# kohjingyu/gill

Hardware: AMD Instinct MI355X
Metric: 512x512 images/sec/node, OPT-6.7B+SD1.5 50-step (higher is better)
Workload: dtype bf16

## Files before the change

### gill_amd/csrc/attention.hip

```cpp
#include "ops.h"
#include <stdlib.h>
#include <type_traits>

#define ATT_KVT 64

template <int DP, int ATT_THREADS>
struct AttCfg {
  static constexpr int KS = DP / 16;
  static constexpr int NDT = (DP + 31) / 32;
  static constexpr int DPV = NDT * 32;
  static constexpr int KSTR = DP + 8;
  static constexpr int VSTR = ATT_KVT + 8;
  static constexpr bool HAS_ONES = (DP % 32) != 0;
  static constexpr int K_CHUNKS = ATT_KVT * DP / 8;
  static constexpr int V_CHUNKS = DPV * ATT_KVT / 8;
  static constexpr int K_PER_THR = (K_CHUNKS + ATT_THREADS - 1) / ATT_THREADS;
  static constexpr int V_PER_THR = (V_CHUNKS + ATT_THREADS - 1) / ATT_THREADS;
  static constexpr int K_ROWS = (K_PER_THR * ATT_THREADS + DP / 8 - 1) / (DP / 8);
  static constexpr int V_ROWS = K_PER_THR * 0 + V_PER_THR * ATT_THREADS / 8;
  static constexpr int K_ELEMS = K_ROWS * KSTR;
  static constexpr int V_ELEMS = V_ROWS * VSTR;
  static constexpr int BUF_ELEMS = K_ELEMS + V_ELEMS;
  static constexpr int SMEM_BYTES = 2 * BUF_ELEMS * 2;
};

template <int DP, int ATT_THREADS>
__global__ __launch_bounds__(ATT_THREADS, (DP <= 64 ? 4 : 2)) void attention_kernel(const AttnArgs p) {
  kernarg_warm<sizeof(AttnArgs)>();
  using Cfg = AttCfg<DP, ATT_THREADS>;
  constexpr int ATT_QB = ATT_THREADS / 2;
  constexpr int KS = Cfg::KS, NDT = Cfg::NDT, KSTR = Cfg::KSTR, VSTR = Cfg::VSTR;
  extern __shared__ __attribute__((aligned(16))) unsigned char att_smem_raw[];
  bf16_t* smem = reinterpret_cast<bf16_t*>(att_smem_raw);

  const int tid = threadIdx.x;
  const int lane = tid & 63;
  const int w = tid >> 6;
  const int nqt = (p.nq + ATT_QB - 1) / ATT_QB;
  int pair, qtile;
  if (p.xcd_map) {
    const int xcd = blockIdx.x & 7, slot = blockIdx.x >> 3;
    pair = xcd + 8 * (slot / nqt);
    qtile = slot - (slot / nqt) * nqt;
  } else {
    pair = blockIdx.x / nqt;
    qtile = blockIdx.x - pair * nqt;
  }
  if (pair >= p.B * p.H) return;
  const int b = pair / p.H, h = pair - b * p.H;
  const int q0 = qtile * ATT_QB + w * 32;
  const bool wave_active = q0 < p.nq;
  const int lq = lane & 31;
  const int hi = lane >> 5;
  const int kvb = p.kv_bstride_zero ? 0 : b;

  const bf16_t* Qb = p.Q + (size_t)(b * p.H + h) * p.nq_pad * DP;
  const bf16_t* Kb = p.K + (size_t)(kvb * p.H + h) * p.nkv_pad * DP;
  const bf16_t* Vb = p.Vt + (size_t)(kvb * p.H + h) * p.dpv * p.nkv_pad;

  int qrow = q0 + lq;
  const bool qvalid = qrow < p.nq;
  if (qrow > p.nq - 1) qrow = p.nq - 1;

  bf16x8 qf[KS];
#pragma unroll
  for (int s = 0; s < KS; ++s) qf[s] = *reinterpret_cast<const bf16x8*>(Qb + (size_t)qrow * DP + s * 16 + hi * 8);

  f32x16 oacc[NDT];
#pragma unroll
  for (int t = 0; t < NDT; ++t)
#pragma unroll
    for (int r = 0; r < 16; ++r) oacc[t][r] = 0.f;

  float m_run = 0.f, l_run = 0.f;

  const int coff = p.nkv - p.nq;
  int kv_end_blk = p.nkv;
  if (p.causal) {
    int lim = qtile * ATT_QB + ATT_QB - 1 + coff + 1;
    if (lim < kv_end_blk) kv_end_blk = lim;
    if (kv_end_blk < 1) kv_end_blk = 1;
  }
  const int ntiles = (kv_end_blk + ATT_KVT - 1) / ATT_KVT;
  const int qidx = qrow + coff;
  const int wave_kv_end = p.causal ? min(p.nkv, q0 + 31 + coff + 1) : p.nkv;

  typedef __attribute__((ext_vector_type(4))) unsigned int u32x4;
  u32x4 kreg[Cfg::K_PER_THR];
  u32x4 vreg[Cfg::V_PER_THR];
// ... 164 lines not shown

template <int DP, int ATT_THREADS>
__global__ __launch_bounds__(ATT_THREADS, 4) void attention_dma_kernel(const AttnArgs p) {
  kernarg_warm<sizeof(AttnArgs)>();
  static_assert(DP == 48, "QF3 needs three padding dims behind d = 40");
  constexpr int NW = ATT_THREADS / 64;
  constexpr int ATT_QB = ATT_THREADS / 2;
  constexpr int KS = DP / 16, NDT = (DP + 31) / 32, NCH = DP / 8;
  constexpr int PPW = 8 / NW;
  constexpr int K_BYTES = 64 * 128, STAGE = 2 * K_BYTES, CONST_OFF = 2 * STAGE;
  extern __shared__ __attribute__((aligned(16))) unsigned char att_smem_raw[];
  unsigned char* smem = att_smem_raw;

  const int tid = threadIdx.x;
  const int lane = tid & 63;
  const int w = __builtin_amdgcn_readfirstlane(tid >> 6);
  const int nqt = p.nq / ATT_QB;
  int pair, qtile;
  if (p.xcd_map) {
    const int xcd = blockIdx.x & 7, slot = blockIdx.x >> 3;
    pair = xcd + 8 * (slot / nqt);
    qtile = slot - (slot / nqt) * nqt;
  } else {
    pair = blockIdx.x / nqt;
    qtile = blockIdx.x - pair * nqt;
  }
  if (pair >= p.B * p.H) return;
  const int b = pair / p.H, h = pair - b * p.H;
  const int q0 = qtile * ATT_QB + w * 32;
  const int lq = lane & 31;
  const int hi = lane >> 5;
  const int kvb = p.kv_bstride_zero ? 0 : b;

  const bf16_t* Qb = p.Q + (size_t)(b * p.H + h) * p.nq_pad * DP;
  const bf16_t* Kb = p.K + (size_t)(kvb * p.H + h) * p.nkv_pad * DP;
  const bf16_t* Vb = p.Vt + (size_t)(kvb * p.H + h) * p.dpv * p.nkv_pad;
  const int qrow = q0 + lq;

  if (tid == 0) *reinterpret_cast<uint4*>(smem + CONST_OFF) = make_uint4(0x3F803F80u, 0x00003F80u, 0u, 0u);

  bf16x8 qf[KS];
#pragma unroll
  for (int s = 0; s < KS; ++s) qf[s] = *reinterpret_cast<const bf16x8*>(Qb + (size_t)qrow * DP + s * 16 + hi * 8);

  const int r8 = lane >> 3, pch = lane & 7;
  unsigned koff[PPW], voff[PPW];
#pragma unroll
  for (int j = 0; j < PPW; ++j) {
    const int i = (w * PPW + j) * 8 + r8;
    const int c = pch ^ ((i >> 1) & 7);
    const int key = (i & ~12) | ((i & 4) << 1) | ((i & 8) >> 1);
    const int ck = c >= NCH ? c - NCH : c;
    koff[j] = (unsigned)((key * DP + ck * 8) * 2);
    voff[j] = (unsigned)((i * p.nkv_pad + c * 8) * 2);
  }
  auto issue_tile = [&](int tile, int stage) {
    const char* kbase = (const char*)(Kb + (size_t)tile * ATT_KVT * DP);
    const char* vbase = (const char*)(Vb + (size_t)tile * ATT_KVT);
    unsigned char* dst = smem + stage * STAGE + (w * PPW) * 1024;
#pragma unroll
    for (int j = 0; j < PPW; ++j) {
      __builtin_amdgcn_global_load_lds((const __attribute__((address_space(1))) void*)(kbase + koff[j]),
                                       (__attribute__((address_space(3))) void*)(dst + j * 1024), 16, 0, 0);
      __builtin_amdgcn_global_load_lds((const __attribute__((address_space(1))) void*)(vbase + voff[j]),
                                       (__attribute__((address_space(3))) void*)(dst + K_BYTES + j * 1024), 16, 0, 0);
    }
  };
// ... 157 lines not shown
static int attention_launch_inst(const AttnArgs& a, hipStream_t s) {
  static bool attr_set = false;
  constexpr int smem = AttCfg<DP, NTHR>::SMEM_BYTES;
  if (!attr_set) {
    GILL_CHECK_HIP(hipFuncSetAttribute((const void*)attention_kernel<DP, NTHR>, hipFuncAttributeMaxDynamicSharedMemorySize, smem));
    attr_set = true;
  }
  constexpr int xcd_on = 1;
  AttnArgs b = a;
  b.xcd_map = xcd_on;
  dim3 grid((xcd_on ? 8 * cdiv(a.H * a.B, 8) : a.H * a.B) * cdiv(a.nq, NTHR / 2), 1, 1);
  hipLaunchKernelGGL((attention_kernel<DP, NTHR>), grid, dim3(NTHR), smem, s, b);
  GILL_CHECK_HIP(hipGetLastError());
  return 0;
}

template <int DP>
static int attention_launch_dp(const AttnArgs& a, hipStream_t s) {
  const int64_t bh = (int64_t)a.H * a.B;
  const bool big = cdiv(a.nq, 256) * bh >= 256;
  if constexpr (DP == 48) {
    if (attention_dma_ok(a, big ? 512 : 256)) return big ? attention_dma_launch<DP, 512>(a, s) : attention_dma_launch<DP, 256>(a, s);
  }
  if (big) return attention_launch_inst<DP, 512>(a, s);
  return attention_launch_inst<DP, 256>(a, s);
}

int attention_launch(const AttnArgs& a, hipStream_t s) {
  GILL_REQUIRE(a.B > 0 && a.H > 0 && a.nq > 0 && a.nkv > 0, "empty attention");
  GILL_REQUIRE(a.nkv_pad % 32 == 0 && a.nkv_pad >= a.nkv, "nkv_pad must be a multiple of 32 covering nkv");
  GILL_REQUIRE(a.nq_pad >= a.nq, "nq_pad must cover nq");
  GILL_REQUIRE(a.dpv >= round_up(a.dp, 32), "dpv must cover roundup(dp, 32)");
  GILL_REQUIRE(a.ldo >= a.H * a.dp, "ldo too small");
  switch (a.dp) {
    case 48:  return attention_launch_dp<48>(a, s);
    case 64:  return attention_launch_dp<64>(a, s);
    case 80:  return attention_launch_dp<80>(a, s);
    case 128: return attention_launch_dp<128>(a, s);
    case 160: return attention_launch_dp<160>(a, s);
    default:
      gill_set_error("attention: unsupported padded head dim (supported: 48, 64, 80, 128, 160)");
      return -2;
  }
}
```

### gill_amd/csrc/ffn.hip

```cpp
#include "ops.h"
#include <type_traits>

namespace {

constexpr int FC = 320;
constexpr int FH = 1280;
constexpr int FTM = 128;
constexpr int FSLOT = 20 * 1024;
constexpr int FNSLOT = 7;
constexpr int FNCH = FH / 64;
constexpr int FBIAS_OFF = FNSLOT * FSLOT;
constexpr int FBO2_OFF = FBIAS_OFF + FNCH * 128 * 4;
constexpr int FW_BYTES = 2560;
constexpr int FSMEM = FBIAS_OFF + FNCH * 128 * 4;
constexpr int FSMEM_PRE = FBO2_OFF + FC * 4;
static_assert(FSMEM_PRE <= 160 * 1024, "LDS budget");
constexpr int FKO = 384;
constexpr int FNPRE = 2 * (FKO / 64);

typedef __attribute__((ext_vector_type(16))) float f32x16;
typedef __attribute__((ext_vector_type(4))) float f32x4;
typedef __attribute__((ext_vector_type(4))) unsigned u32x4;
typedef __attribute__((ext_vector_type(2))) unsigned u32x2;

template <int N> __device__ __forceinline__ void ffn_wait_vm() {
  __builtin_amdgcn_s_waitcnt((N & 15) | ((N >> 4) << 14) | (7 << 4) | (15 << 8));
}

struct Slab { const bf16_t* src; int ld; };

template <bool PRE>
__global__ __launch_bounds__(256) __attribute__((amdgpu_waves_per_eu(1, 1))) void ffn_fused_kernel(const FfnArgs p) {
  kernarg_warm<sizeof(FfnArgs)>();
  constexpr int SB = PRE ? FNPRE % 7 : 0;
  extern __shared__ __attribute__((aligned(16))) unsigned char smem[];
  const int tid = threadIdx.x, lane = tid & 63;
  const int w = __builtin_amdgcn_readfirstlane(tid >> 6);
  const int l31 = lane & 31, hi = lane >> 5;
  const int m = blockIdx.x * FTM + w * 32 + l31;

  const int srow = lane >> 3, schunk = (lane & 7) ^ srow;
  auto slab_f = [&](int f) -> Slab {
    if constexpr (PRE) return Slab{p.Wpp + (size_t)(f / 5) * 160 * FC + 64 * (f % 5), FC};
    else return Slab{p.Wfo + (size_t)(f / 5) * 160 * (5 * FC) + 4 * FC + 64 * (f % 5), 5 * FC};
  };
  auto slab_g = [&](int g) -> Slab { return Slab{p.Wo + (size_t)(g / 6) * 160 * FKO + 64 * (g % 6), FKO}; };
  auto slab_c = [&](int c, int q) -> Slab {
    if (q < 5) return Slab{p.W1c + (size_t)c * 128 * FC + 64 * q, FC};
    return Slab{p.W2p + (size_t)(q - 5) * 160 * FH + 64 * c, FH};
  };
  auto issue_piece = [&](const Slab& st, int slot, int i) {
    const int pc = w + 4 * i;
    const uint64_t b64 = (uint64_t)(uintptr_t)(st.src + (size_t)(8 * pc) * st.ld);
    const bf16_t* base = (const bf16_t*)(uintptr_t)(((uint64_t)(unsigned)__builtin_amdgcn_readfirstlane((unsigned)(b64 >> 32)) << 32) |
                                                     (uint64_t)(unsigned)__builtin_amdgcn_readfirstlane((unsigned)b64));
    const bf16_t* src = (const bf16_t*)((const char*)base + (unsigned)((srow * st.ld + schunk * 8) * 2));
    __builtin_amdgcn_global_load_lds((const __attribute__((address_space(1))) void*)src,
                                     (__attribute__((address_space(3))) void*)(smem + slot * FSLOT + pc * 1024), 16, 0, 0);
  };
  auto wfrag = [&](const unsigned char* slot, int tile, int s) -> bf16x8 {
    const int row = tile * 32 + l31;
    return *reinterpret_cast<const bf16x8*>(slot + row * 128 + (((2 * s + hi) ^ (row & 7)) * 16));
  };

#pragma unroll
  for (int f = 0; f < 6; ++f) {
    const Slab st = PRE ? slab_g(f) : slab_f(f);
#pragma unroll
    for (int i = 0; i < 5; ++i) issue_piece(st, f, i);
  }
  __builtin_amdgcn_sched_barrier(0);
  bf16x8 tf[20];
  float ln_mean, ln_rstd;
  bf16x8 xf[PRE ? FKO / 16 : 1];
  u32x4 res[PRE ? 20 : 1];
  if constexpr (PRE) {
    const bf16_t* tsrc = p.T + (size_t)(blockIdx.x * FTM + w * 32 + (lane >> 2)) * FC + (lane & 3) * 8;
#pragma unroll
    for (int i = 0; i < 10; ++i) {
      res[2 * i] = *reinterpret_cast<const u32x4*>(tsrc + 32 * i);
      res[2 * i + 1] = *reinterpret_cast<const u32x4*>(tsrc + 32 * i + 16 * FC);
    }
#pragma unroll
    for (int s = 0; s < FKO / 16; ++s) xf[s] = *reinterpret_cast<const bf16x8*>(p.X + (size_t)m * FKO + 16 * s + 8 * hi);
  } else {
#pragma unroll
    for (int s = 0; s < 20; ++s) tf[s] = *reinterpret_cast<const bf16x8*>(p.T + (size_t)m * FC + 16 * s + 8 * hi);
    const int R = p.ln_rows ? p.ln_rows : p.M;
    const int mr = m >= R ? m - R : m;
    const float* base = p.ln_stats + (size_t)mr * 2;
    const size_t pstride = (size_t)R * 2;
    float2 st = make_float2(0.f, 0.f);
    for (int pl = 0; pl < p.ln_planes; ++pl) {
      const float2 v = *reinterpret_cast<const float2*>(base + (size_t)pl * pstride);
      st.x += v.x; st.y += v.y;
    }
    ln_mean = st.x * (1.f / FC);
    const float var = fmaxf(st.y * (1.f / FC) - ln_mean * ln_mean, 0.f);
    ln_rstd = rsqrtf(var + p.ln_eps);
  }
  {
    float* bt = reinterpret_cast<float*>(smem + FBIAS_OFF);
    static_assert(FNCH * 128 % 256 == 0, "table fill: whole rounds of the workgroup");
    float tb[FNCH * 128 / 256];
#pragma unroll
    for (int j = 0; j < FNCH * 128 / 256; ++j) tb[j] = p.b1c[tid + 256 * j];
#pragma unroll
    for (int j = 0; j < FNCH * 128 / 256; ++j) bt[tid + 256 * j] = tb[j];
    if constexpr (PRE) {
      float* b2t = reinterpret_cast<float*>(smem + FBO2_OFF);
// ... 176 lines not shown
          const f32x4 bg = *reinterpret_cast<const f32x4*>(btab + c * 128 + 64 + tt * 32 + 16 * hh + 8 * g2 + 4 * hi);
          const int r = 8 * hh + 4 * g2;
          const float o0 = (acc[tt][r] + bv.x) * gelu_logistic(acc[2 + tt][r] + bg.x);
          const float o1 = (acc[tt][r + 1] + bv.y) * gelu_logistic(acc[2 + tt][r + 1] + bg.y);
          const float o2 = (acc[tt][r + 2] + bv.z) * gelu_logistic(acc[2 + tt][r + 2] + bg.z);
          const float o3 = (acc[tt][r + 3] + bv.w) * gelu_logistic(acc[2 + tt][r + 3] + bg.w);
          pk.u[2 * g2] = pack_bf2(o0, o1);
          pk.u[2 * g2 + 1] = pack_bf2(o2, o3);
        }
        pf[2 * tt + hh] = pk.v;
      }
#define S2_STAGE(U, N, NL)                                                                                                      \
    {                                                                                                                            \
      auto mma = [&](int s, const bf16x8* wfp) {                                                                                 \
        _Pragma("unroll") for (int q = 0; q < 5; ++q)                                                                           \
          out[5 * (U) + q] = __builtin_amdgcn_mfma_f32_32x32x16_bf16(wfp[q], pf[s], out[5 * (U) + q], 0, 0, 0);                  \
      };                                                                                                                         \
      const Slab nx = slab_c(LAST ? c : c + 1, 4 + (U));                                                                         \
      run_stage(I5{}, std::integral_constant<int, (U) == 0 ? 5 : (LAST ? 0 : 4)>{}, std::integral_constant<int, LAST ? NL : N>{},\
                std::integral_constant<int, LAST ? 0 : ((U) == 1 ? 5 : 4)>{}, (SB + 8 + (U)) % 7, (SB + 9 + (U)) % 7, nx,        \
                (SB + 7 + (U)) % 7, mma, std::false_type{});                                                                     \
    }
    S2_STAGE(0, 19, 0) S2_STAGE(1, 19, 0)
#undef S2_STAGE
  };
  for (int c = 0; c + 1 < FNCH; ++c) run_chunk(c, std::false_type{});
  run_chunk(FNCH - 1, std::true_type{});

  constexpr int OSTR = 656;
  __syncthreads();
  unsigned char* wtile = smem + (size_t)(w * 32) * OSTR;
  unsigned char* otile = wtile + (size_t)l31 * OSTR;
  {
    const bf16_t* rsrc = p.resid + (size_t)(blockIdx.x * FTM + w * 32) * FC;
    u32x4 rr[20];
#pragma unroll
    for (int j = 0; j < 20; ++j) rr[j] = *reinterpret_cast<const u32x4*>(rsrc + (size_t)(lane + 64 * j) * 8);
#pragma unroll
    for (int j = 0; j < 20; ++j) {
      const int c = lane + 64 * j;
      *reinterpret_cast<u32x4*>(wtile + (c / 40) * OSTR + (c % 40) * 16) = rr[j];
    }
  }
#pragma unroll
  for (int i = 0; i < 10; ++i) {
#pragma unroll
    for (int q4 = 0; q4 < 4; ++q4) {
      const int n = i * 32 + 8 * q4 + 4 * hi;
      const f32x4 bo = *reinterpret_cast<const f32x4*>(p.bo + n);
      const u32x2 rv = *reinterpret_cast<const u32x2*>(otile + n * 2);
      const float v0 = out[i][4 * q4] + bo.x + __uint_as_float(rv.x << 16);
      const float v1 = out[i][4 * q4 + 1] + bo.y + __uint_as_float(rv.x & 0xffff0000u);
      const float v2 = out[i][4 * q4 + 2] + bo.z + __uint_as_float(rv.y << 16);
      const float v3 = out[i][4 * q4 + 3] + bo.w + __uint_as_float(rv.y & 0xffff0000u);
      *reinterpret_cast<u32x2*>(otile + n * 2) = u32x2{pack_bf2(v0, v1), pack_bf2(v2, v3)};
    }
  }
  {
    bf16_t* odst = p.out + (size_t)(blockIdx.x * FTM + w * 32) * FC;
#pragma unroll
    for (int j = 0; j < 20; ++j) {
      const int c = lane + 64 * j;
      *reinterpret_cast<u32x4*>(odst + (size_t)c * 8) = *reinterpret_cast<const u32x4*>(wtile + (c / 40) * OSTR + (c % 40) * 16);
    }
  }
  if (p.gn_stats) {
    __syncthreads();
// ... 37 lines not shown
      const int src = (h / 16) * 32 + gate * 16 + (h % 16);
      W1c[i] = wff1[(size_t)src * FC + (Wpp ? perm16(k) : k)];
      if (k == 0) b1c[row] = bff1[src];
    } else if (i < n1 + n2) {
      const int64_t t = i - n1;
      const int pos = (int)(t % FH), n = (int)(t / FH);
      W2p[t] = wfo[(size_t)n * (5 * FC) + perm16(pos)];
    } else {
      const int64_t t = i - n1 - n2;
      const int pos = (int)(t % FC), n = (int)(t / FC);
      Wpp[t] = wfo[(size_t)n * (5 * FC) + 4 * FC + perm16(pos)];
    }
  }
}

}

bool ffn_fused_supported(int C, int M) { return C == FC && M % FTM == 0 && M > 0; }

int ffn_relayout_launch(const bf16_t* wff1, const float* bff1, const bf16_t* wfo, bf16_t* W1c, float* b1c, bf16_t* W2p, bf16_t* Wpp,
                        hipStream_t s) {
  hipLaunchKernelGGL(ffn_relayout_kernel, dim3(1024), dim3(256), 0, s, wff1, bff1, wfo, W1c, b1c, W2p, Wpp);
  GILL_CHECK_HIP(hipGetLastError());
  return 0;
}

int ffn_fused_launch(const FfnArgs& a, hipStream_t s) {
  GILL_REQUIRE(ffn_fused_supported(FC, a.M), "fused feed-forward block: M must be a multiple of 128");
  GILL_REQUIRE(a.T && a.W1c && a.b1c && a.W2p && a.bo && a.resid && a.out, "fused feed-forward block: null operand");
  GILL_REQUIRE(!a.gn_stats || (a.rows_per_batch > 0 && a.rows_per_batch % 128 == 0), "fused feed-forward block: GroupNorm partials need whole 64-row slabs per sample");
  const bool pre = a.X != nullptr;
  if (pre) {
    GILL_REQUIRE(a.Wo && a.bo2 && a.Wpp, "fused feed-forward block with attn2.to_out in front: null operand");
  } else {
    GILL_REQUIRE(a.Wfo && a.ln_stats && a.ln_planes >= 1, "fused feed-forward block: LayerNorm row-sum planes missing");
  }
  static bool attr_set[2] = {false, false};
  const void* fn = pre ? (const void*)ffn_fused_kernel<true> : (const void*)ffn_fused_kernel<false>;
  const int smem = pre ? FSMEM_PRE : FSMEM;
  if (!attr_set[pre]) {
    GILL_CHECK_HIP(hipFuncSetAttribute(fn, hipFuncAttributeMaxDynamicSharedMemorySize, smem));
    attr_set[pre] = true;
  }
  if (pre) hipLaunchKernelGGL(ffn_fused_kernel<true>, dim3(a.M / FTM), dim3(256), smem, s, a);
  else hipLaunchKernelGGL(ffn_fused_kernel<false>, dim3(a.M / FTM), dim3(256), smem, s, a);
  GILL_CHECK_HIP(hipGetLastError());
  return 0;
}
```

### gill_amd/csrc/ops.h

```cpp
#pragma once
#include "common.h"

enum { ACT_NONE = 0, ACT_RELU = 1, ACT_GELU = 2, ACT_SILU = 3, ACT_GEGLU = 4, ACT_QUICK_GELU = 5  };
enum { OUT_BF16 = 0, OUT_F32 = 1, OUT_QKV = 2, OUT_SOFTMAX80 = 3 };

struct GemmArgs {
  int M = 0, N = 0, K = 0;
  const bf16_t* A = nullptr;  int lda = 0;
  const bf16_t* A2 = nullptr; int lda2 = 0;
  int K1 = 0;
  int conv = 0;
  int IH = 0, IW = 0, OH = 0, OW = 0, Cin = 0, stride = 1, ups = 0;
  const bf16_t* X1 = nullptr; const bf16_t* X2 = nullptr; int KX = 0, KX1 = 0;
  const bf16_t* W = nullptr;
  int k_chunked = 0;
  float alpha = 1.f;
  const float* bias = nullptr;
  const float* rowvec = nullptr; int rows_per_batch = 1; int rowvec_bstride = 0;
  const void* resid = nullptr; int ldr = 0; int resid_f32 = 0;
  int act = ACT_NONE;
  int out_mode = OUT_BF16;
  void* C = nullptr; int ldc = 0;
  bf16_t* Cq = nullptr; bf16_t* Ck = nullptr; bf16_t* Cvt = nullptr;
  int heads = 0, dp = 0, dpv = 0, ntok = 0, ntok_pad_q = 0, ntok_pad_kv = 0, seg_base = 0;
// ... 43 lines not shown
  bf16_t* C = nullptr;
  float* gn_stats = nullptr; int gn_groups = 0; int gn_cg = 0;
  int splitk = 1; float* ws = nullptr;
};
int conv3x3_fp8_launch(const ConvF8Args& a, hipStream_t s);

#define F8_LIN_ACT_SCALE 16.0f
struct LinF8Args {
  int M = 0, N = 0, K = 0;
  const unsigned char* A8 = nullptr;
  const unsigned char* W8 = nullptr;
  const float* colscale = nullptr;
  const float* bias = nullptr;
  bf16_t* C = nullptr;
};
int geglu_fp8_launch(const LinF8Args& a, hipStream_t s);
int linear_weight_quant_fp8_launch(const bf16_t* w, int N, int K, float act_scale, unsigned char* w8, float* colscale, hipStream_t s);
int ln_quant_fp8_launch(const bf16_t* t, int M, int C, const float* ln_stats, int planes, int ln_rows, float eps, float act_scale, unsigned char* y,
                        hipStream_t s);
int conv_fp8_kpad(int Cin);
int quant_bf16_fp8_launch(const bf16_t* x, float scale, int64_t n, unsigned char* y, hipStream_t s);
int conv_weight_quant_fp8_launch(const void* w_oihw, int dtype, int Cout, int Cin, float act_scale, unsigned char* w8, float* colscale,
                                 hipStream_t s);

struct AttnArgs {
  const bf16_t* Q = nullptr; const bf16_t* K = nullptr; const bf16_t* Vt = nullptr; bf16_t* O = nullptr;
  int B = 0, H = 0, nq = 0, nkv = 0, nq_pad = 0, nkv_pad = 0, dp = 0, dpv = 0;
  int ldo = 0;
  float scale = 1.f;
  int d = 0;
  int causal = 0;
  int kv_bstride_zero = 0;
  int xcd_map = 1;
};
int attention_launch(const AttnArgs& a, hipStream_t s);


struct FfnArgs {
  int M = 0;
  const bf16_t* T = nullptr;
  const float* ln_stats = nullptr; int ln_planes = 0, ln_rows = 0; float ln_eps = 1e-5f;
  const bf16_t* W1c = nullptr; const float* b1c = nullptr;
  const bf16_t* W2p = nullptr;
  const bf16_t* Wfo = nullptr; const float* bo = nullptr;
  const bf16_t* resid = nullptr; bf16_t* out = nullptr;
  float* gn_stats = nullptr; int rows_per_batch = 0;
  const bf16_t* X = nullptr;
  const bf16_t* Wo = nullptr; const float* bo2 = nullptr;
  const bf16_t* Wpp = nullptr;
};
bool ffn_fused_supported(int C, int M);
int ffn_relayout_launch(const bf16_t* wff1, const float* bff1, const bf16_t* wfo, bf16_t* W1c, float* b1c, bf16_t* W2p, bf16_t* Wpp,
                        hipStream_t s);
int ffn_fused_launch(const FfnArgs& a, hipStream_t s);

struct LnProjArgs {
  int mode = 0;
  int M = 0;
  const bf16_t* X = nullptr;
  bf16_t* T = nullptr;
  const bf16_t* W1 = nullptr;
  const float* b1 = nullptr;
  const bf16_t* W2p = nullptr;
  const float* c2 = nullptr;
  float ln_eps = 1e-5f;
  bf16_t *Cq = nullptr, *Ck = nullptr, *Cvt = nullptr;
  int heads = 0, dp = 0, dpv = 0, ntok = 0, ntok_pad = 0, seg_base = 0;
  float qscale = 1.f;
  const float* gn_ss = nullptr;
};
bool lnproj_supported(int C, int M, int heads, int dp);
int lnproj_kperm_launch(const bf16_t* src, int N, bf16_t* dst, hipStream_t s);
int lnproj_launch(const LnProjArgs& a, hipStream_t s);

int layernorm_launch(const void* x, int x_f32, const float* gamma, const float* beta, bf16_t* y,
                     int rows, int C, float eps, hipStream_t s);
int layernorm_f32out_launch(const void* x, int x_f32, const float* gamma, const float* beta, float* y,
                            int rows, int C, float eps, hipStream_t s);

#define GN_STATS_ROWS 32
static inline size_t groupnorm_stats_floats(int B, int HW, int groups) {
  return (size_t)B * ((HW + GN_STATS_ROWS - 1) / GN_STATS_ROWS) * groups * 2 + (size_t)B * groups * 2;
// ... 100 lines not shown
```

### gill_amd/csrc/unet.hip

```cpp
#include "engine_util.h"
#include <math.h>
#include <stdlib.h>
#include <map>
#include <set>
#include <hip/hip_fp16.h>

namespace {

struct ConvW {
  bf16_t* w = nullptr; float* b = nullptr; int cin = 0, cout = 0; int chunked = 0;  int ups4 = 0;
  unsigned char* w8 = nullptr; float* cs = nullptr; int kpad = 0;
};
struct LinW { bf16_t* w = nullptr; float* b = nullptr; int out = 0, in = 0; };
struct NormW { float* g = nullptr; float* b = nullptr; int c = 0; };

struct ResnetW {
  NormW n1, n2;
  ConvW c1, c2;
  bool has_sc = false;
  LinW sc;
  bf16_t* c2f_w = nullptr; float* c2f_b = nullptr;
  int cin = 0, cout = 0, temb_off = 0;
};

// ... 210 lines not shown
    for (int c = threadIdx.x * 8; c < C; c += 2048) *reinterpret_cast<uint4*>(dst + c) = make_uint4(0, 0, 0, 0);
  }
#pragma unroll
  for (int o = 32; o > 0; o >>= 1) { sum += __shfl_xor(sum, o, 64); dot += __shfl_xor(dot, o, 64); }
  if ((threadIdx.x & 63) == 0) { red[0][threadIdx.x >> 6] = sum; red[1][threadIdx.x >> 6] = dot; }
  __syncthreads();
  if (threadIdx.x == 0) {
    cs[blockIdx.x] = red[0][0] + red[0][1] + red[0][2] + red[0][3];
    cb[blockIdx.x] = j < ctx_len ? red[1][0] + red[1][1] + red[1][2] + red[1][3] : -1e30f;
  }
}
__global__ __launch_bounds__(256) void xalg_values_operand_kernel(const bf16_t* __restrict__ T, int H, int C, int ctx_len, bf16_t* __restrict__ Wo) {
  __shared__ bf16_t tile[80][66];
  const int cb = blockIdx.x % (C / 64), h = (blockIdx.x / (C / 64)) % H, b = blockIdx.x / ((C / 64) * H);
  for (int i = threadIdx.x; i < 80 * 64; i += 256) {
    const int j = i >> 6, c = i & 63;
    tile[j][c] = j < ctx_len ? T[(size_t)(b * ctx_len + j) * (2 * H * C) + (size_t)H * C + (size_t)h * C + cb * 64 + c] : (bf16_t)0;
  }
  __syncthreads();
  for (int i = threadIdx.x; i < 64 * 80; i += 256) {
    const int c = i / 80, j = i - c * 80;
    Wo[((size_t)b * C + cb * 64 + c) * (80 * H) + h * 80 + j] = tile[j][c];
  }
}

static bool lnproj_on() {
  static const bool on = [] { const char* e = getenv("GILL_UNET_LNPROJ"); return !(e && e[0] == '0'); }();
  return on;
}
static bool xalg_on() {
  static const bool on = [] { const char* e = getenv("GILL_UNET_XALG"); return !(e && e[0] == '0'); }();
  return on;
}
static bool ffn_fused_on() {
  static const bool on = [] { const char* e = getenv("GILL_UNET_FFN_FUSED"); return !(e && e[0] == '0'); }();
  return on;
}

namespace {

struct Loader {
  const WeightTable& wt;
  DevPool& pool;
  hipStream_t s;
  int ctx_len = 0;
  int norm(const std::string& p, int c, NormW* n) {
    n->c = c;
    GILL_TRY(load_f32(wt, pool, p + ".weight", c, &n->g, s));
    return load_f32(wt, pool, p + ".bias", c, &n->b, s);
  }
  int conv3(const std::string& p, int cin, int cout, int hw, ConvW* c, bool f8 = false, bool ups4 = false) {
    c->cin = cin; c->cout = cout; c->chunked = conv_k_chunked(hw, cin, cout) ? 1 : 0;
    const gill_tensor* t;
    GILL_TRY(wt.get(p + ".weight", (int64_t)cout * cin * 9, &t));
    static const int ups4_on = [] { const char* v = getenv("GILL_CONV_UPS4"); return v ? atoi(v) : 1; }();
    if (ups4 && ups4_on && !f8) {
      c->ups4 = 1; c->chunked = 0;
      GILL_TRY(pool.alloc(&c->w, (size_t)16 * cout * cin, false));
      GILL_TRY(conv_weight_relayout_ups4_launch(t->data, t->dtype, cout, cin, c->w, s));
      return load_f32(wt, pool, p + ".bias", cout, &c->b, s);
    }
    if (f8) {
      c->kpad = conv_fp8_kpad(cin);
      GILL_TRY(pool.alloc(&c->w8, (size_t)cout * c->kpad, false));
      GILL_TRY(pool.alloc(&c->cs, (size_t)cout, false));
      GILL_TRY(conv_weight_quant_fp8_launch(t->data, t->dtype, cout, cin, F8_ACT_SCALE, c->w8, c->cs, s));
// ... 438 lines not shown
        resid = out->p;
      }
      GILL_TRY(conv8(n2, w.c2, nullptr, 0, resid, *out));
      m->arena.release(mk);
      return 0;
    }
    Tensor n1 = talloc(H, Wd, w.cin);
    if (pre && !x2) n1 = *pre;
    else GILL_TRY(gnorm(x1, x2, w.n1, 1e-5f, 1, n1));
    Tensor h = talloc(H, Wd, w.cout, true);
    Tensor n2 = talloc(H, Wd, w.cout);
    FusedNorm f2{&w.n2, 1e-5f, 1, n2, false, false};
    GILL_TRY(conv(n1, nullptr, w.c1, 1, 0, temb_rows ? temb_rows + w.temb_off : nullptr, temb_bstride, nullptr, h, &f2));
    if (!f2.done) GILL_TRY(gnorm(h, nullptr, w.n2, 1e-5f, 1, n2));
    if (w.has_sc) {
      GemmArgs g;
      g.conv = 1; g.IH = H; g.IW = Wd; g.OH = H; g.OW = Wd; g.Cin = w.cout; g.stride = 1; g.ups = 0;
      g.M = Bx * H * Wd; g.N = w.cout; g.K = 9 * w.cout + w.cin;
      g.A = n2.p; g.K1 = w.cout;
      g.X1 = x1.p; g.X2 = x2 ? x2->p : nullptr; g.KX = w.cin; g.KX1 = x1.C;
      g.W = w.c2f_w; g.bias = w.c2f_b; g.k_chunked = w.c2.chunked;
      g.rows_per_batch = H * Wd;
      g.C = out->p; g.ldc = w.cout;
      fuse_stats(g, *out);
      GILL_TRY(gemm(g, nullptr, out, next));
    } else {
      GILL_TRY(conv(n2, nullptr, w.c2, 1, 0, nullptr, 0, x1.p, *out, next));
    }
    m->arena.release(mk);
    return 0;
  }

  int attend(const bf16_t* q, const bf16_t* k, const bf16_t* vt, bf16_t* o, int nq, int nkv, int nq_pad, int nkv_pad,
             const XfW& w) {
    if (dry) return 0;
    AttnArgs a;
    a.Q = q; a.K = k; a.Vt = vt; a.O = o;
    a.B = Bx; a.H = w.heads; a.nq = nq; a.nkv = nkv; a.nq_pad = nq_pad; a.nkv_pad = nkv_pad;
    a.dp = w.dp; a.dpv = w.dpv; a.ldo = w.heads * w.dp; a.d = w.d;
    a.scale = 1.0f / sqrtf((float)w.d);
    return attention_launch(a, s);
  }

  bool xf_wants_table(const XfW& w, int HW, bool shared) const {
    return w.wqkv1p != nullptr && !shared && lnproj_supported(w.C, Bx * HW, w.heads, w.dp) && HW % 128 == 0;
  }

  int xf(const Tensor& x, const XfW& w, Tensor* out, bool out_stats, bool shared = false, const Tensor* pre = nullptr,
         FusedNorm* next = nullptr, const float* pre_ss = nullptr) {
    const int Bpre = Bx, Bfull = shared ? 2 * Bx : Bx;
    Bx = Bfull;
    const int H = x.H, Wd = x.W, C = w.C, HW = H * Wd, M = Bfull * HW, M1 = Bpre * HW;
    const int nh = w.heads, hdp = nh * w.dp;
    const bool ffn_fused = w.w1c != nullptr && ffn_fused_supported(C, M) && HW % 128 == 0;
    const bool lnproj = w.wqkv1p != nullptr && !shared && lnproj_supported(C, M, nh, w.dp) && HW % 32 == 0;
    *out = talloc(H, Wd, C, out_stats);
    const size_t mk = m->arena.mark();
    Tensor n = talloc(H, Wd, C);
    Tensor xd = x;
    if (shared) xd = talloc(H, Wd, C);
    Bx = Bpre;
    float* gn_ss = nullptr;
    bool gn_folded = false;
    if (lnproj && HW % 128 == 0) gn_ss = (float*)m->arena.alloc(sizeof(float) * (size_t)Bx * 2 * C);
    if (pre_ss && gn_ss) { gn_ss = const_cast<float*>(pre_ss); gn_folded = true; }
    else if (pre) n = *pre;
    else GILL_TRY(gnorm(x, nullptr, w.gn, 1e-6f, 0, n, 0.f, gn_ss, &gn_folded));
    Bx = Bfull;
    Tensor t = talloc(H, Wd, C);
    RowStats st1 = ln_slot(M, C), st2 = ln_slot(M, C), st3 = ln_slot(M, C);
    if (!lnproj) GILL_TRY(linear(n.p, C, nullptr, 0, C, M1, w.proj_in.w, w.proj_in.b, C, C, nullptr, ACT_NONE, t.p, C, nullptr, &st1));
    const int hw_pad = round_up(HW, 32);
    bf16_t* q = (bf16_t*)m->arena.alloc(sizeof(bf16_t) * (size_t)Bx * nh * hw_pad * w.dp);
    bf16_t* k = (bf16_t*)m->arena.alloc(sizeof(bf16_t) * (size_t)Bx * nh * hw_pad * w.dp);
    bf16_t* vt = (bf16_t*)m->arena.alloc(sizeof(bf16_t) * (size_t)Bx * nh * w.dpv * hw_pad);
    bf16_t* o = (bf16_t*)m->arena.alloc(sizeof(bf16_t) * (size_t)M * hdp);
    LnProjArgs lp;
    lp.M = M; lp.T = t.p; lp.heads = nh; lp.dp = w.dp; lp.dpv = w.dpv; lp.ntok = HW; lp.ntok_pad = hw_pad;
    lp.Cq = q; lp.Ck = k; lp.Cvt = vt; lp.qscale = 1.4426950408889634f / sqrtf((float)w.d);
    if (lnproj) {
      lp.mode = 0; lp.X = gn_folded ? x.p : n.p; lp.gn_ss = gn_folded ? gn_ss : nullptr; lp.W1 = w.proj_in.w; lp.b1 = w.proj_in.b; lp.W2p = w.wqkv1p; lp.c2 = w.c_qkv1;
      if (!dry) GILL_TRY(lnproj_launch(lp, s));
    } else {
      GemmArgs g;
      g.M = M1; g.N = 3 * hdp; g.K = C; g.K1 = C; g.A = t.p; g.lda = C; g.W = w.wqkv1;
      g.ln_stats = st1.p; g.ln_planes = st1.planes; g.ln_colsum = w.s_qkv1; g.bias = w.c_qkv1;
      g.out_mode = OUT_QKV; g.Cq = q; g.Ck = k; g.Cvt = vt; g.heads = nh; g.dp = w.dp; g.dpv = w.dpv;
      g.ntok = HW; g.ntok_pad_q = hw_pad; g.ntok_pad_kv = hw_pad; g.seg_base = 0;
      g.qscale = 1.4426950408889634f / sqrtf((float)w.d);
      GILL_TRY(gemm(g));
    }
    Bx = Bpre;
    GILL_TRY(attend(q, k, vt, o, HW, HW, hw_pad, hw_pad, w));
    Bx = Bfull;
    const bf16_t* tres = t.p;
    bool ffn_pre = false;
    bool xalg_done = false;
    {
    if (lnproj) {
      GILL_REQUIRE(!w.xg, "internal: the fused projection pairs and the two-GEMM cross-attention are alternatives");
      lp.mode = 1; lp.X = o; lp.gn_ss = nullptr; lp.W1 = w.out1.w; lp.b1 = w.out1.b; lp.W2p = w.wq2p; lp.c2 = w.c_q2;
      if (!dry) GILL_TRY(lnproj_launch(lp, s));
    } else {
    GILL_TRY(linear(o, hdp, nullptr, 0, hdp, M1, w.out1.w, w.out1.b, C, hdp, t.p, ACT_NONE, t.p, C, nullptr, &st2));
    if (shared && !dry) {
      GILL_TRY(dup_pair_launch(t.p, x.p, xd.p, sizeof(bf16_t) * (size_t)M1 * C, s));
    }
    if (w.xg) {
      const int n80 = 80 * nh, id = w.layer_id;
      GemmArgs g;
      g.M = M; g.N = n80; g.K = C; g.K1 = C; g.A = t.p; g.lda = C; g.W = m->xq_w[id];
      g.wb_rows = HW; g.wb_stride = (int64_t)n80 * C; g.vb_stride = n80;
      g.ln_stats = st2.p; g.ln_planes = st2.planes; g.ln_rows = M1; g.ln_colsum = m->xq_cs[id]; g.bias = m->xq_b[id];
      g.out_mode = OUT_SOFTMAX80; g.C = o; g.ldc = n80;
      GILL_TRY(gemm(g));
      GemmArgs g2;
      g2.M = M; g2.N = C; g2.K = n80; g2.K1 = n80; g2.A = o; g2.lda = n80; g2.W = m->xo_w[id]; g2.bias = w.out2.b;
      g2.wb_rows = HW; g2.wb_stride = (int64_t)n80 * C;
      g2.resid = t.p; g2.ldr = C; g2.C = t.p; g2.ldc = C;
      GILL_TRY(gemm(g2, &st3));
      xalg_done = true;
    } else {
      GemmArgs g;
      g.M = M; g.N = hdp; g.K = C; g.K1 = C; g.A = t.p; g.lda = C; g.W = w.wq2;
      g.ln_stats = st2.p; g.ln_planes = st2.planes; g.ln_rows = M1; g.ln_colsum = w.s_q2; g.bias = w.c_q2;
      g.out_mode = OUT_QKV; g.Cq = q; g.Ck = k; g.Cvt = vt; g.heads = nh; g.dp = w.dp; g.dpv = w.dpv;
      g.ntok = HW; g.ntok_pad_q = hw_pad; g.ntok_pad_kv = hw_pad; g.seg_base = 0;
      g.qscale = 1.4426950408889634f / sqrtf((float)w.d);
      GILL_TRY(gemm(g));
    }
    }
    if (!xalg_done) {
    GILL_REQUIRE(m->kcache[w.layer_id] != nullptr || dry, "internal: cross-attention K/V cache missing");
    GILL_TRY(attend(q, m->kcache[w.layer_id], m->vcache[w.layer_id], o, HW, m->cfg.ctx_len, hw_pad, m->ctx_pad, w));
    ffn_pre = ffn_fused && w.wpp != nullptr;
    GILL_REQUIRE(!ffn_fused || ffn_pre == w.w1c_kperm, "internal: fused feed-forward kernel form does not match the layout its weights were written in");
    if (!ffn_pre) GILL_TRY(linear(o, hdp, nullptr, 0, hdp, M, w.out2.w, w.out2.b, C, hdp, t.p, ACT_NONE, t.p, C, nullptr, &st3));
    }
    }
    if (ffn_fused) {
      if (!dry) {
        FfnArgs fa;
        fa.M = M; fa.T = tres; fa.ln_stats = st3.p; fa.ln_planes = st3.planes;
        fa.W1c = w.w1c; fa.b1c = w.b1c; fa.W2p = w.w2p; fa.Wfo = w.wfo; fa.bo = w.bfo; fa.resid = xd.p; fa.out = out->p;
        if (ffn_pre) { fa.X = o; fa.Wo = w.out2.w; fa.bo2 = w.out2.b; fa.Wpp = w.wpp; }
        if (out->stats && out->sbin == 5) { fa.gn_stats = out->stats; fa.rows_per_batch = HW; out->nslab = HW / GN_SLAB_ROWS; }
        else out->stats = nullptr;
        GILL_TRY(ffn_fused_launch(fa, s));
      }
      m->arena.release(mk);
      return 0;
    }
    bf16_t* ffh = (bf16_t*)m->arena.alloc(sizeof(bf16_t) * (size_t)M * 4 * C);
    unsigned char* t8 = w.wff1_8 ? (unsigned char*)m->arena.alloc((size_t)M * C) : nullptr;
    if (w.wff1_8) {
      if (!dry) {
        GILL_TRY(ln_quant_fp8_launch(tres, M, C, st3.p, st3.planes, 0, 1e-5f, F8_LIN_ACT_SCALE, t8, s));
        LinF8Args a;
        a.M = M; a.N = 8 * C; a.K = C; a.A8 = t8; a.W8 = w.wff1_8; a.colscale = w.cs_ff1; a.bias = w.bff1; a.C = ffh;
        GILL_TRY(geglu_fp8_launch(a, s));
        GILL_TRY(dbg_sync("geglu fp8", M, 8 * C, C));
      }
    } else {
      GemmArgs g;
      g.M = M; g.N = 8 * C; g.K = C; g.K1 = C; g.A = tres; g.lda = C; g.W = w.wff1; g.bias = w.bff1;
      g.ln_stats = st3.p; g.ln_planes = st3.planes; g.ln_colsum = w.s_ff1;
      g.act = ACT_GEGLU; g.C = ffh; g.ldc = 4 * C;
      GILL_TRY(gemm(g));
    }
    GILL_TRY(linear(ffh, 4 * C, tres, C, 4 * C, M, w.wfo, w.bfo, C, 5 * C, xd.p, ACT_NONE, out->p, C, out, nullptr, next));
    m->arena.release(mk);
    return 0;
  }

  int forward(const float* sample, float* eps_out) {
    const gill_unet_config& c = m->cfg;
    const int* ch = c.block_out_channels;
    const int L = c.sample_size;
// ... 597 lines not shown
```

Before: 8.832.

## Share prefix Q projection across duplicated batch halves in cross-attention blocks

When the transformer block runs on a batch whose two halves share an identical prefix (classifier-free guidance style duplication), it computes the attn2 Q projection only for the first half. The attention kernels remap Q reads for the second half onto the first, and the fused FFN kernel reads the residual and T rows from the first half as well. This removes the dup_pair copy and half of the Q GEMM. It adds index remapping and new preconditions on batch layout, and it is on by default behind an environment toggle.

```diff
diff --git a/gill_amd/csrc/attention.hip b/gill_amd/csrc/attention.hip
--- a/gill_amd/csrc/attention.hip
+++ b/gill_amd/csrc/attention.hip
@@ -54,7 +54,8 @@
   const int hi = lane >> 5;
   const int kvb = p.kv_bstride_zero ? 0 : b;
 
-  const bf16_t* Qb = p.Q + (size_t)(b * p.H + h) * p.nq_pad * DP;
+  const int qb = (p.q_samples > 0 && b >= p.q_samples) ? b - p.q_samples : b;
+  const bf16_t* Qb = p.Q + (size_t)(qb * p.H + h) * p.nq_pad * DP;
   const bf16_t* Kb = p.K + (size_t)(kvb * p.H + h) * p.nkv_pad * DP;
   const bf16_t* Vb = p.Vt + (size_t)(kvb * p.H + h) * p.dpv * p.nkv_pad;
 
@@ -285,7 +286,8 @@
   const int hi = lane >> 5;
   const int kvb = p.kv_bstride_zero ? 0 : b;
 
-  const bf16_t* Qb = p.Q + (size_t)(b * p.H + h) * p.nq_pad * DP;
+  const int qb = (p.q_samples > 0 && b >= p.q_samples) ? b - p.q_samples : b;
+  const bf16_t* Qb = p.Q + (size_t)(qb * p.H + h) * p.nq_pad * DP;
   const bf16_t* Kb = p.K + (size_t)(kvb * p.H + h) * p.nkv_pad * DP;
   const bf16_t* Vb = p.Vt + (size_t)(kvb * p.H + h) * p.dpv * p.nkv_pad;
   const int qrow = q0 + lq;
@@ -509,6 +511,7 @@
   GILL_REQUIRE(a.nq_pad >= a.nq, "nq_pad must cover nq");
   GILL_REQUIRE(a.dpv >= round_up(a.dp, 32), "dpv must cover roundup(dp, 32)");
   GILL_REQUIRE(a.ldo >= a.H * a.dp, "ldo too small");
+  GILL_REQUIRE(a.q_samples == 0 || (a.q_samples > 0 && a.B <= 2 * a.q_samples), "q_samples must cover at least half of the batch");
   switch (a.dp) {
     case 48:  return attention_launch_dp<48>(a, s);
     case 64:  return attention_launch_dp<64>(a, s);
diff --git a/gill_amd/csrc/ffn.hip b/gill_amd/csrc/ffn.hip
--- a/gill_amd/csrc/ffn.hip
+++ b/gill_amd/csrc/ffn.hip
@@ -38,6 +38,7 @@
   const int w = __builtin_amdgcn_readfirstlane(tid >> 6);
   const int l31 = lane & 31, hi = lane >> 5;
   const int m = blockIdx.x * FTM + w * 32 + l31;
+  const int ms0 = (p.src_rows > 0 && (int)blockIdx.x * FTM >= p.src_rows) ? blockIdx.x * FTM - p.src_rows : blockIdx.x * FTM;
 
   const int srow = lane >> 3, schunk = (lane & 7) ^ srow;
   auto slab_f = [&](int f) -> Slab {
@@ -75,7 +76,7 @@
   bf16x8 xf[PRE ? FKO / 16 : 1];
   u32x4 res[PRE ? 20 : 1];
   if constexpr (PRE) {
-    const bf16_t* tsrc = p.T + (size_t)(blockIdx.x * FTM + w * 32 + (lane >> 2)) * FC + (lane & 3) * 8;
+    const bf16_t* tsrc = p.T + (size_t)(ms0 + w * 32 + (lane >> 2)) * FC + (lane & 3) * 8;
 #pragma unroll
     for (int i = 0; i < 10; ++i) {
       res[2 * i] = *reinterpret_cast<const u32x4*>(tsrc + 32 * i);
@@ -318,7 +319,7 @@
   unsigned char* wtile = smem + (size_t)(w * 32) * OSTR;
   unsigned char* otile = wtile + (size_t)l31 * OSTR;
   {
-    const bf16_t* rsrc = p.resid + (size_t)(blockIdx.x * FTM + w * 32) * FC;
+    const bf16_t* rsrc = p.resid + (size_t)(ms0 + w * 32) * FC;
     u32x4 rr[20];
 #pragma unroll
     for (int j = 0; j < 20; ++j) rr[j] = *reinterpret_cast<const u32x4*>(rsrc + (size_t)(lane + 64 * j) * 8);
@@ -422,8 +423,10 @@
   const bool pre = a.X != nullptr;
   if (pre) {
     GILL_REQUIRE(a.Wo && a.bo2 && a.Wpp, "fused feed-forward block with attn2.to_out in front: null operand");
+    GILL_REQUIRE(a.src_rows == 0 || (a.src_rows > 0 && a.src_rows % FTM == 0 && a.M <= 2 * a.src_rows), "fused feed-forward block: src_rows must be whole tiles covering half of M");
   } else {
     GILL_REQUIRE(a.Wfo && a.ln_stats && a.ln_planes >= 1, "fused feed-forward block: LayerNorm row-sum planes missing");
+    GILL_REQUIRE(a.src_rows == 0, "fused feed-forward block: src_rows needs attn2.to_out in front (X)");
   }
   static bool attr_set[2] = {false, false};
   const void* fn = pre ? (const void*)ffn_fused_kernel<true> : (const void*)ffn_fused_kernel<false>;
diff --git a/gill_amd/csrc/ops.h b/gill_amd/csrc/ops.h
--- a/gill_amd/csrc/ops.h
+++ b/gill_amd/csrc/ops.h
@@ -99,6 +99,7 @@
   int causal = 0;
   int kv_bstride_zero = 0;
   int xcd_map = 1;
+  int q_samples = 0;
 };
 int attention_launch(const AttnArgs& a, hipStream_t s);
 
@@ -115,6 +116,7 @@
   const bf16_t* X = nullptr;
   const bf16_t* Wo = nullptr; const float* bo2 = nullptr;
   const bf16_t* Wpp = nullptr;
+  int src_rows = 0;
 };
 bool ffn_fused_supported(int C, int M);
 int ffn_relayout_launch(const bf16_t* wff1, const float* bff1, const bf16_t* wfo, bf16_t* W1c, float* b1c, bf16_t* W2p, bf16_t* Wpp,
diff --git a/gill_amd/csrc/unet.hip b/gill_amd/csrc/unet.hip
--- a/gill_amd/csrc/unet.hip
+++ b/gill_amd/csrc/unet.hip
@@ -266,6 +266,10 @@
   static const bool on = [] { const char* e = getenv("GILL_UNET_XALG"); return !(e && e[0] == '0'); }();
   return on;
 }
+static bool edges_on() {
+  static const bool on = [] { const char* e = getenv("GILL_UNET_EDGES"); return !(e && e[0] == '0'); }();
+  return on;
+}
 static bool ffn_fused_on() {
   static const bool on = [] { const char* e = getenv("GILL_UNET_FFN_FUSED"); return !(e && e[0] == '0'); }();
   return on;
@@ -770,9 +774,10 @@
   }
 
   int attend(const bf16_t* q, const bf16_t* k, const bf16_t* vt, bf16_t* o, int nq, int nkv, int nq_pad, int nkv_pad,
-             const XfW& w) {
+             const XfW& w, int q_samples = 0) {
     if (dry) return 0;
     AttnArgs a;
+    a.q_samples = q_samples;
     a.Q = q; a.K = k; a.Vt = vt; a.O = o;
     a.B = Bx; a.H = w.heads; a.nq = nq; a.nkv = nkv; a.nq_pad = nq_pad; a.nkv_pad = nkv_pad;
     a.dp = w.dp; a.dpv = w.dpv; a.ldo = w.heads * w.dp; a.d = w.d;
@@ -792,6 +797,7 @@
     const int nh = w.heads, hdp = nh * w.dp;
     const bool ffn_fused = w.w1c != nullptr && ffn_fused_supported(C, M) && HW % 128 == 0;
     const bool lnproj = w.wqkv1p != nullptr && !shared && lnproj_supported(C, M, nh, w.dp) && HW % 32 == 0;
+    const bool share_q = shared && edges_on() && !w.xg && ffn_fused && w.wpp != nullptr;
     *out = talloc(H, Wd, C, out_stats);
     const size_t mk = m->arena.mark();
     Tensor n = talloc(H, Wd, C);
@@ -841,7 +847,7 @@
       if (!dry) GILL_TRY(lnproj_launch(lp, s));
     } else {
     GILL_TRY(linear(o, hdp, nullptr, 0, hdp, M1, w.out1.w, w.out1.b, C, hdp, t.p, ACT_NONE, t.p, C, nullptr, &st2));
-    if (shared && !dry) {
+    if (shared && !share_q && !dry) {
       GILL_TRY(dup_pair_launch(t.p, x.p, xd.p, sizeof(bf16_t) * (size_t)M1 * C, s));
     }
     if (w.xg) {
@@ -860,7 +866,7 @@
       xalg_done = true;
     } else {
       GemmArgs g;
-      g.M = M; g.N = hdp; g.K = C; g.K1 = C; g.A = t.p; g.lda = C; g.W = w.wq2;
+      g.M = share_q ? M1 : M; g.N = hdp; g.K = C; g.K1 = C; g.A = t.p; g.lda = C; g.W = w.wq2;
       g.ln_stats = st2.p; g.ln_planes = st2.planes; g.ln_rows = M1; g.ln_colsum = w.s_q2; g.bias = w.c_q2;
       g.out_mode = OUT_QKV; g.Cq = q; g.Ck = k; g.Cvt = vt; g.heads = nh; g.dp = w.dp; g.dpv = w.dpv;
       g.ntok = HW; g.ntok_pad_q = hw_pad; g.ntok_pad_kv = hw_pad; g.seg_base = 0;
@@ -870,8 +876,9 @@
     }
     if (!xalg_done) {
     GILL_REQUIRE(m->kcache[w.layer_id] != nullptr || dry, "internal: cross-attention K/V cache missing");
-    GILL_TRY(attend(q, m->kcache[w.layer_id], m->vcache[w.layer_id], o, HW, m->cfg.ctx_len, hw_pad, m->ctx_pad, w));
+    GILL_TRY(attend(q, m->kcache[w.layer_id], m->vcache[w.layer_id], o, HW, m->cfg.ctx_len, hw_pad, m->ctx_pad, w, share_q ? Bpre : 0));
     ffn_pre = ffn_fused && w.wpp != nullptr;
+    GILL_REQUIRE(!share_q || ffn_pre, "internal: the shared prefix ran past attn2.to_q without the feed-forward kernel form that reads it");
     GILL_REQUIRE(!ffn_fused || ffn_pre == w.w1c_kperm, "internal: fused feed-forward kernel form does not match the layout its weights were written in");
     if (!ffn_pre) GILL_TRY(linear(o, hdp, nullptr, 0, hdp, M, w.out2.w, w.out2.b, C, hdp, t.p, ACT_NONE, t.p, C, nullptr, &st3));
     }
@@ -882,6 +889,7 @@
         fa.M = M; fa.T = tres; fa.ln_stats = st3.p; fa.ln_planes = st3.planes;
         fa.W1c = w.w1c; fa.b1c = w.b1c; fa.W2p = w.w2p; fa.Wfo = w.wfo; fa.bo = w.bfo; fa.resid = xd.p; fa.out = out->p;
         if (ffn_pre) { fa.X = o; fa.Wo = w.out2.w; fa.bo2 = w.out2.b; fa.Wpp = w.wpp; }
+        if (share_q) { fa.src_rows = M1; fa.resid = x.p; }
         if (out->stats && out->sbin == 5) { fa.gn_stats = out->stats; fa.rows_per_batch = HW; out->nslab = HW / GN_SLAB_ROWS; }
         else out->stats = nullptr;
         GILL_TRY(ffn_fused_launch(fa, s));
```

Result: no change. 8.865 (median of 6 runs) (+0.4%).
